# uc-vision/splat-trainer

Measured on AMD Instinct MI355X. Metric: fwd+bwd Gaussians/s, higher is better.
Workload: dtype f32

## Files before the change

### splat-trainer_amd/csrc/composite.hip

```cpp
#include "gsr_device.h"
#include "gsr_dpp_reduce.h"
#include "../../include/gsplat_hip.h"

namespace {

inline GsrRasterParams to_params(const GsrRasterParamsC* c) {
  GsrRasterParams rp;
  __builtin_memcpy(&rp, c, sizeof(rp));
  return rp;
}

typedef float v2f __attribute__((ext_vector_type(2)));
struct __attribute__((packed, aligned(4))) Rank4 { uint32_t x, y, z, w; };
#define GSR_V2(x) ((v2f){(x), (x)})

__device__ __forceinline__ v2f eval_q2(v2f dx, float dy, float A, float B, float C) {
#pragma clang fp contract(off)
  const float t = (B + B) * dy;
  const float u = (C * dy) * dy;
  return __builtin_elementwise_fma(dx * A, dx, __builtin_elementwise_fma(GSR_V2(t), dx, GSR_V2(u)));
}
__device__ __forceinline__ void eval_qt(v2f dx, float dy, float A, float B, float C, v2f& q, v2f& tx, v2f& ty) {
#pragma clang fp contract(off)
  const float bdy = B * dy, cdy = C * dy;
  tx = __builtin_elementwise_fma(dx, GSR_V2(A), GSR_V2(bdy));
  ty = __builtin_elementwise_fma(dx, GSR_V2(B), GSR_V2(cdy));
  q = eval_q2(dx, dy, A, B, C);
}
__device__ __forceinline__ v2f eval_alpha2(v2f q, float l2op) {
#pragma clang fp contract(off)
  const v2f e = __builtin_elementwise_fma(q, GSR_V2(-0.72134752044448170368f), GSR_V2(l2op));
  return (v2f){__builtin_amdgcn_exp2f(e.x), __builtin_amdgcn_exp2f(e.y)};
}
__device__ __forceinline__ v2f eval_G2(v2f q) {
#pragma clang fp contract(off)
  const v2f e = q * -0.72134752044448170368f;
  return (v2f){__builtin_amdgcn_exp2f(e.x), __builtin_amdgcn_exp2f(e.y)};
}

__device__ __forceinline__ v2f clamp_alpha2(v2f a, float cmax) {
  return (v2f){__builtin_amdgcn_fmed3f(a.x, 0.f, cmax), __builtin_amdgcn_fmed3f(a.y, 0.f, cmax)};
}

struct Splat {
  float u, v, A, B, C, op, qlim, f0, f1, f2, depth, l2op;
  uint32_t halves;
};

template <int C, bool DEPTH = false>
__device__ __forceinline__ Splat load_splat_packed(const float* __restrict__ rec, uint32_t packed) {
  const uint32_t k = packed & 0x3FFFFFFFu;
  const float4* r = reinterpret_cast<const float4*>(rec + (size_t)GSR_ROW_FLOATS * k);
  const float4 r0 = r[0], r1 = r[1];
  Splat s;
  s.u = r0.x; s.v = r0.y; s.A = r0.z; s.B = r0.w; s.C = r1.x; s.op = r1.y; s.qlim = r1.z; s.f0 = r1.w;
  s.f1 = 0.f; s.f2 = 0.f; s.depth = 0.f; s.l2op = 0.f;
  s.halves = packed >> 30;
  if (C > 1 || DEPTH) { const float4 r2 = r[2]; s.f1 = r2.x; s.f2 = r2.y; s.depth = r2.z; s.l2op = r2.w; }
  return s;
}

template <int C, bool DEPTH = false>
__device__ __forceinline__ Splat load_splat(const float* __restrict__ rec, const uint32_t* __restrict__ sorted_rank,
                                            uint32_t i) {
  const uint32_t packed = (uint32_t)__builtin_amdgcn_readfirstlane((int)sorted_rank[i]);
  const uint32_t k = packed & 0x3FFFFFFFu;
  const float4* r = reinterpret_cast<const float4*>(rec + (size_t)GSR_ROW_FLOATS * k);
  const float4 r0 = r[0], r1 = r[1];
  Splat s;
  s.u = r0.x; s.v = r0.y; s.A = r0.z; s.B = r0.w; s.C = r1.x; s.op = r1.y; s.qlim = r1.z; s.f0 = r1.w;
  s.f1 = 0.f; s.f2 = 0.f; s.depth = 0.f; s.l2op = 0.f;
  s.halves = packed >> 30;
  if (C > 1 || DEPTH) { const float4 r2 = r[2]; s.f1 = r2.x; s.f2 = r2.y; s.depth = r2.z; s.l2op = r2.w; }
  return s;
}

#define GSR_SEG_HEAVY 0x80000000u

struct SegDev {
  const uint32_t* tile_seg;
  const uint32_t* seg_desc;
  const uint32_t* seg_total;
  const uint32_t* tile_order;
  float* seg_P;
  float4* seg_TC;
  int* seg_last;
  float* seg_median;
};

#define GSR_TILE_CLASSES 32
#define GSR_TILE_GROUP 16
#define GSR_SEG_CLASS_COUNT(band) (16u + GSR_TILE_CLASSES * (band))
__host__ __device__ inline int gsr_tile_band(int t, int n) { (void)n; return (t / GSR_TILE_GROUP) & 7; }
__host__ __device__ inline int gsr_tile_band_stride(int n) {
  return (n + 8 * GSR_TILE_GROUP - 1) / (8 * GSR_TILE_GROUP) * GSR_TILE_GROUP;
}

__device__ __forceinline__ int ordered_tile(const SegDev& seg, int num_tiles, uint32_t b, int lane) {
  const uint32_t band = b & 7u, t = b >> 3;
  uint32_t upto = lane < GSR_TILE_CLASSES ? seg.seg_total[GSR_SEG_CLASS_COUNT(band) + (GSR_TILE_CLASSES - 1 - lane)] : 0u;
#pragma unroll
  for (int o = 1; o < GSR_TILE_CLASSES; o <<= 1) {
    const uint32_t below = (uint32_t)__shfl_up((int)upto, o, 64);
    if (lane >= o) upto += below;
  }
  const uint64_t longer = __ballot(lane < GSR_TILE_CLASSES && t < upto);
  if (longer == 0ull) return -1;
  const int l = __builtin_ctzll(longer);
  const uint32_t before = l ? (uint32_t)__builtin_amdgcn_readlane((int)upto, l - 1) : 0u;
  return (int)seg.tile_order[((size_t)band * GSR_TILE_CLASSES + (size_t)(GSR_TILE_CLASSES - 1 - l)) *
                                 (size_t)gsr_tile_band_stride(num_tiles) + (t - before)];
}

template <int C>
struct FwdPix {
  v2f T2[2], col2[2][3], med2[2];
  int lastc[4];
  uint32_t pf_rank, pf_bits, pf_sink;
};

constexpr int GSR_K6_PREFETCH = 32;
template <int C, bool PF>
__device__ __forceinline__ void fwd_prefetch_init(FwdPix<C>& px, const uint32_t* __restrict__ sorted_rank,
                                                  uint32_t tile_start, uint32_t begin, uint32_t pf_end, int lane) {
  px.pf_bits = 0u; px.pf_sink = 0u; px.pf_rank = 0u;
  if (!PF) return;
  const uint32_t first = tile_start + ((begin - tile_start + GSR_K6_PREFETCH - 1u) & ~(uint32_t)(GSR_K6_PREFETCH - 1));
  const uint32_t p = first + GSR_K6_PREFETCH + (uint32_t)lane;
  if (lane < GSR_K6_PREFETCH && p < pf_end) px.pf_rank = sorted_rank[p];
}
template <int C>
__device__ __forceinline__ void fwd_prefetch_step(FwdPix<C>& px, const float* __restrict__ rec,
                                                  const uint32_t* __restrict__ sorted_rank, uint32_t i, uint32_t pf_end,
                                                  int lane) {
  px.pf_sink |= px.pf_bits;
  const uint32_t p1 = i + GSR_K6_PREFETCH + (uint32_t)lane, p2 = p1 + GSR_K6_PREFETCH;
  const bool mine = lane < GSR_K6_PREFETCH;
  px.pf_bits = (mine && p1 < pf_end)
                   ? __float_as_uint(rec[(size_t)GSR_ROW_FLOATS * (px.pf_rank & 0x3FFFFFFFu)]) : 0u;
  px.pf_rank = (mine && p2 < pf_end) ? sorted_rank[p2] : 0u;
}

template <int C, bool VIS, bool MEDIAN, bool PF>
__device__ __forceinline__ void fwd_walk(FwdPix<C>& px, const float* __restrict__ rec,
                                         const uint32_t* __restrict__ sorted_rank,
                                         const uint32_t* __restrict__ sorted_inst, uint32_t tile_start, uint32_t begin,
                                         uint32_t end, float fx0, float fy0, const GsrRasterParams& rp, int lane,
                                         float* __restrict__ vis_partial, float* __restrict__ pair_vis,
                                         uint32_t pf_end) {
  const uint32_t vis_slot = (uint32_t)(((lane >> 4) & 1) * 2 + (lane >> 5));
  if (begin >= end) return;
  uint32_t rk[4] = {0u, 0u, 0u, 0u}, rk_next[4] = {0u, 0u, 0u, 0u};
  Splat nxt;
  if constexpr (PF) {
    const Rank4 q4 = *reinterpret_cast<const Rank4*>(sorted_rank + begin);
    rk[0] = (uint32_t)__builtin_amdgcn_readfirstlane((int)q4.x); rk[1] = (uint32_t)__builtin_amdgcn_readfirstlane((int)q4.y);
    rk[2] = (uint32_t)__builtin_amdgcn_readfirstlane((int)q4.z); rk[3] = (uint32_t)__builtin_amdgcn_readfirstlane((int)q4.w);
    nxt = load_splat_packed<C, MEDIAN>(rec, rk[0]);
  } else {
    nxt = load_splat<C, MEDIAN>(rec, sorted_rank, begin);
  }
  for (uint32_t i = begin; i < end; i += 4) {
    if (PF && ((i - tile_start) & (GSR_K6_PREFETCH - 1)) == 0u) fwd_prefetch_step<C>(px, rec, sorted_rank, i, pf_end, lane);
    if constexpr (PF) {
      if (i + 4 < end) {
        const Rank4 q4 = *reinterpret_cast<const Rank4*>(sorted_rank + i + 4);
        rk_next[0] = (uint32_t)__builtin_amdgcn_readfirstlane((int)q4.x); rk_next[1] = (uint32_t)__builtin_amdgcn_readfirstlane((int)q4.y);
        rk_next[2] = (uint32_t)__builtin_amdgcn_readfirstlane((int)q4.z); rk_next[3] = (uint32_t)__builtin_amdgcn_readfirstlane((int)q4.w);
      }
    }
    float wq[4] = {0.f, 0.f, 0.f, 0.f};
#pragma unroll
    for (int m = 0; m < 4; ++m) {
      if (i + m < end) {
        const Splat s = nxt;
        if constexpr (PF) {
          if (i + m + 1 < end) nxt = load_splat_packed<C, MEDIAN>(rec, m < 3 ? rk[m + 1] : rk_next[0]);
        } else {
          nxt = load_splat<C, MEDIAN>(rec, sorted_rank, min(i + m + 1, end - 1u));
        }
        const v2f dx2 = (v2f){fx0, fx0 + 8.f} - GSR_V2(s.u);
        const int idx = (int)(i - tile_start) + m + 1;
        v2f wsum2 = GSR_V2(0.f);
#pragma unroll
        for (int h = 0; h < 2; ++h) {
          if (!(s.halves & (1u << h))) continue;
          const float dy = (h ? fy0 + 8.f : fy0) - s.v;
          const v2f q = eval_q2(dx2, dy, s.A, s.B, s.C);
          const bool hit0 = px.T2[h].x >= rp.T_eps && q.x <= s.qlim;
          const bool hit1 = px.T2[h].y >= rp.T_eps && q.y <= s.qlim;
          if (__ballot(hit0 || hit1) != 0ull) {
            const v2f G = eval_G2(q);
            const v2f a_raw = G * s.op;
            v2f alpha = clamp_alpha2(a_raw, rp.clamp_max_alpha);
            alpha = (v2f){hit0 ? alpha.x : 0.f, hit1 ? alpha.y : 0.f};
            const v2f w = alpha * px.T2[h];
            px.col2[h][0] = __builtin_elementwise_fma(w, GSR_V2(s.f0), px.col2[h][0]);
            if (C > 1) px.col2[h][1] = __builtin_elementwise_fma(w, GSR_V2(s.f1), px.col2[h][1]);
            if (C > 2) px.col2[h][2] = __builtin_elementwise_fma(w, GSR_V2(s.f2), px.col2[h][2]);
            wsum2 += w;
            px.T2[h] = px.T2[h] - w;
            if (hit0) px.lastc[2 * h] = idx;
            if (hit1) px.lastc[2 * h + 1] = idx;
            if (MEDIAN) {
              if (hit0 && px.med2[h].x == 0.f && px.T2[h].x < 0.5f) px.med2[h].x = s.depth;
              if (hit1 && px.med2[h].y == 0.f && px.T2[h].y < 0.5f) px.med2[h].y = s.depth;
            }
          }
        }
        wq[m] = wsum2.x + wsum2.y;
      }
    }
    if (VIS) {
      float r = gsr_swap16_add(gsr_swap32_add(wq[0], wq[1]), gsr_swap32_add(wq[2], wq[3]));
      r = gsr_row_sum_to_lane15(r);
      const uint32_t pos = i + vis_slot;
      if ((lane & 15) == 15 && pos < end) {
        pair_vis[pos] = r;
        if (r > 0.f) vis_partial[sorted_inst[pos]] = r;
      }
    }
    const bool live = px.T2[0].x >= rp.T_eps || px.T2[0].y >= rp.T_eps || px.T2[1].x >= rp.T_eps ||
                      px.T2[1].y >= rp.T_eps;
    if (__ballot(live) == 0ull) break;
    if constexpr (PF) { rk[0] = rk_next[0]; rk[1] = rk_next[1]; rk[2] = rk_next[2]; rk[3] = rk_next[3]; }
  }
}

template <int C>
__device__ __forceinline__ void fwd_init(FwdPix<C>& px, int px0, int py0, int W, int H) {
#pragma unroll
  for (int h = 0; h < 2; ++h) {
    const bool in_y = (py0 + 8 * h) < H;
    px.T2[h] = (v2f){(in_y && px0 < W) ? 1.f : 0.f, (in_y && (px0 + 8) < W) ? 1.f : 0.f};
    px.med2[h] = GSR_V2(0.f);
    px.col2[h][0] = px.col2[h][1] = px.col2[h][2] = GSR_V2(0.f);
  }
#pragma unroll
  for (int p = 0; p < 4; ++p) px.lastc[p] = 0;
}

template <int C>
__device__ __forceinline__ void seg_alpha_pass(uint32_t sidx, const float* __restrict__ rec,
                                               const uint32_t* __restrict__ sorted_rank, int tiles_x,
                                               const GsrRasterParams& rp, const SegDev& seg) {
  const uint32_t* d = seg.seg_desc + 4 * (size_t)sidx;
  const int tile = (int)d[0];
  const uint32_t begin = d[1], end = d[2];
  const int lane = (int)threadIdx.x;
  const int tx = tile % tiles_x, ty = tile / tiles_x;
  const float fx0 = (float)(tx * 16 + (lane & 7)) + 0.5f, fy0 = (float)(ty * 16 + (lane >> 3)) + 0.5f;
  v2f P2[2] = {GSR_V2(1.f), GSR_V2(1.f)};
  Splat nxt = load_splat<1>(rec, sorted_rank, begin);
  for (uint32_t i = begin; i < end; ++i) {
    const Splat s = nxt;
    if (i + 1 < end) nxt = load_splat<1>(rec, sorted_rank, i + 1);
    const v2f dx2 = (v2f){fx0, fx0 + 8.f} - GSR_V2(s.u);
#pragma unroll
    for (int h = 0; h < 2; ++h) {
      if (!(s.halves & (1u << h))) continue;
      const float dy = (h ? fy0 + 8.f : fy0) - s.v;
      const v2f q = eval_q2(dx2, dy, s.A, s.B, s.C);
      const bool in0 = q.x <= s.qlim, in1 = q.y <= s.qlim;
      if (__ballot(in0 || in1) != 0ull) {
        v2f alpha = clamp_alpha2(eval_G2(q) * s.op, rp.clamp_max_alpha);
        alpha = (v2f){in0 ? alpha.x : 0.f, in1 ? alpha.y : 0.f};
        P2[h] = P2[h] - alpha * P2[h];
      }
    }
  }
  float* out = seg.seg_P + 256 * (size_t)sidx + lane;
  out[0] = P2[0].x; out[64] = P2[0].y; out[128] = P2[1].x; out[192] = P2[1].y;
}

template <int C, bool VIS, bool MEDIAN, bool PF>
__global__ __launch_bounds__(64) void composite_fwd_kernel(const float* __restrict__ rec,
                                                           const uint32_t* __restrict__ sorted_rank,
                                                           const uint32_t* __restrict__ sorted_inst,
                                                           const uint32_t* __restrict__ tile_range, int W, int H,
                                                           int tiles_x, int num_tiles, GsrRasterParams rp,
                                                           float* __restrict__ image, float* __restrict__ final_T,
                                                           int* __restrict__ last, float* __restrict__ median,
                                                           float* __restrict__ vis_partial,
                                                           float* __restrict__ pair_vis, SegDev seg, int tile_blocks) {
  if ((int)blockIdx.x >= tile_blocks) {
    const uint32_t h = blockIdx.x - (uint32_t)tile_blocks;
    if (h < seg.seg_total[1]) {
      const uint32_t sidx = (seg.tile_seg + 2 * (size_t)num_tiles)[h];
      if (sidx != 0xFFFFFFFFu) {
        const uint32_t* d = seg.seg_desc + 4 * (size_t)sidx;
        if (d[1] < d[2]) seg_alpha_pass<C>(sidx, rec, sorted_rank, tiles_x, rp, seg);
      }
    }
    return;
  }
  const int lane = (int)threadIdx.x;
  int tile;
  if (seg.tile_order) {
    tile = ordered_tile(seg, num_tiles, blockIdx.x, lane);
    if (tile < 0) return;
  } else {
    tile = gsr_xcd_remap((int)blockIdx.x, num_tiles);
  }
  const uint32_t tseg = seg.tile_seg ? seg.tile_seg[2 * tile + 1] : 0u;
  if (tseg & GSR_SEG_HEAVY) return;
  const int tx = tile % tiles_x, ty = tile / tiles_x;
  const int px0 = tx * 16 + (lane & 7), py0 = ty * 16 + (lane >> 3);
  const float fx0 = (float)px0 + 0.5f, fy0 = (float)py0 + 0.5f;
  const uint32_t start = tile_range[2 * tile], end = tile_range[2 * tile + 1];

  FwdPix<C> px;
  fwd_init<C>(px, px0, py0, W, H);
  fwd_prefetch_init<C, PF>(px, sorted_rank, start, start, end, lane);
  if (tseg == 0u) {
    fwd_walk<C, VIS, MEDIAN, PF>(px, rec, sorted_rank, sorted_inst, start, start, end, fx0, fy0, rp, lane, vis_partial,
                             pair_vis, end);
  } else {
    const uint32_t first = seg.tile_seg[2 * tile];
    for (uint32_t j = 0; j < tseg; ++j) {
      const uint32_t* d = seg.seg_desc + 4 * (size_t)(first + j);
      fwd_walk<C, VIS, MEDIAN, PF>(px, rec, sorted_rank, sorted_inst, start, d[1], d[2], fx0, fy0, rp, lane, vis_partial,
                               pair_vis, end);
      float4* out = seg.seg_TC + 256 * (size_t)(first + j) + lane;
#pragma unroll
      for (int p = 0; p < 4; ++p) {
        const int h = p >> 1;
        out[64 * p] = (p & 1) ? make_float4(px.T2[h].y, px.col2[h][0].y, px.col2[h][1].y, px.col2[h][2].y)
                              : make_float4(px.T2[h].x, px.col2[h][0].x, px.col2[h][1].x, px.col2[h][2].x);
      }
      const bool live = px.T2[0].x >= rp.T_eps || px.T2[0].y >= rp.T_eps || px.T2[1].x >= rp.T_eps ||
                        px.T2[1].y >= rp.T_eps;
      if (__ballot(live) == 0ull) break;
    }
  }

  if (PF && (px.pf_sink | px.pf_bits) == 0x7FC0FFEEu) final_T[0] = 0.f;
#pragma unroll
  for (int p = 0; p < 4; ++p) {
    const int x = px0 + 8 * (p & 1), y = py0 + 8 * (p >> 1);
    if (x < W && y < H) {
      const size_t pix = (size_t)y * W + x;
      const int h = p >> 1;
#pragma unroll
      for (int c = 0; c < C; ++c) image[pix * C + c] = (p & 1) ? px.col2[h][c].y : px.col2[h][c].x;
      final_T[pix] = (p & 1) ? px.T2[h].y : px.T2[h].x;
      last[pix] = px.lastc[p];
      if (MEDIAN) median[pix] = (p & 1) ? px.med2[h].y : px.med2[h].x;
    }
  }
}

template <int C, bool VIS, bool MEDIAN, bool PF>
__global__ __launch_bounds__(64) void seg_composite_kernel(const float* __restrict__ rec,
                                                           const uint32_t* __restrict__ sorted_rank,
                                                           const uint32_t* __restrict__ sorted_inst,
                                                           const uint32_t* __restrict__ tile_range, int W, int H,
                                                           int tiles_x, int num_tiles, GsrRasterParams rp,
                                                           float* __restrict__ vis_partial,
                                                           float* __restrict__ pair_vis, SegDev seg) {
  if (blockIdx.x >= seg.seg_total[1]) return;
  const uint32_t sidx = (seg.tile_seg + 2 * (size_t)num_tiles)[blockIdx.x];
  if (sidx == 0xFFFFFFFFu) return;
  const uint32_t* d = seg.seg_desc + 4 * (size_t)sidx;
  const int tile = (int)d[0];
  const uint32_t begin = d[1], end = d[2];
  const uint32_t first = seg.tile_seg[2 * tile];
  const int lane = (int)threadIdx.x;
  const int tx = tile % tiles_x, ty = tile / tiles_x;
  const int px0 = tx * 16 + (lane & 7), py0 = ty * 16 + (lane >> 3);
  const float fx0 = (float)px0 + 0.5f, fy0 = (float)py0 + 0.5f;

  FwdPix<C> px;
  fwd_init<C>(px, px0, py0, W, H);
  fwd_prefetch_init<C, PF>(px, sorted_rank, tile_range[2 * tile], begin, end, lane);
  for (uint32_t s = first; s < sidx; ++s) {
    const float* P = seg.seg_P + 256 * (size_t)s + lane;
    px.T2[0] = px.T2[0] * (v2f){P[0], P[64]};
    px.T2[1] = px.T2[1] * (v2f){P[128], P[192]};
  }
  const bool alive[4] = {px.T2[0].x >= rp.T_eps, px.T2[0].y >= rp.T_eps, px.T2[1].x >= rp.T_eps, px.T2[1].y >= rp.T_eps};
  if (__ballot(alive[0] || alive[1] || alive[2] || alive[3]) != 0ull)
    fwd_walk<C, VIS, MEDIAN, PF>(px, rec, sorted_rank, sorted_inst, tile_range[2 * tile], begin, end, fx0, fy0, rp, lane,
                             vis_partial, pair_vis, end);
  const size_t o = 256 * (size_t)sidx + lane;
#pragma unroll
  for (int p = 0; p < 4; ++p) {
    const int h = p >> 1;
    const float t = (p & 1) ? px.T2[h].y : px.T2[h].x;
    seg.seg_TC[o + 64 * p] = (p & 1) ? make_float4(alive[p] ? t : -1.f, px.col2[h][0].y, px.col2[h][1].y, px.col2[h][2].y)
                                     : make_float4(alive[p] ? t : -1.f, px.col2[h][0].x, px.col2[h][1].x, px.col2[h][2].x);
    seg.seg_last[o + 64 * p] = px.lastc[p];
    if (MEDIAN) seg.seg_median[o + 64 * p] = (p & 1) ? px.med2[h].y : px.med2[h].x;
  }
}

template <int C, bool MEDIAN>
__global__ __launch_bounds__(64) void seg_combine_kernel(int W, int H, int tiles_x, int num_tiles,
                                                         float* __restrict__ image, float* __restrict__ final_T,
                                                         int* __restrict__ last, float* __restrict__ median,
                                                         SegDev seg) {
  const int tile = (int)blockIdx.x;
  const uint32_t tseg = seg.tile_seg[2 * tile + 1];
  if (!(tseg & GSR_SEG_HEAVY)) return;
  const uint32_t n = tseg & ~GSR_SEG_HEAVY;
  const uint32_t first = seg.tile_seg[2 * tile];
  const int lane = (int)threadIdx.x;
  const int tx = tile % tiles_x, ty = tile / tiles_x;
  const int px0 = tx * 16 + (lane & 7), py0 = ty * 16 + (lane >> 3);
  float col[4][3], T[4], med[4];
  int lastc[4];
#pragma unroll
  for (int p = 0; p < 4; ++p) {
    col[p][0] = col[p][1] = col[p][2] = 0.f;
    T[p] = 1.f; med[p] = 0.f; lastc[p] = 0;
  }
  for (uint32_t j = 0; j < n; ++j) {
    const size_t s = first + j, o = 256 * s + lane;
#pragma unroll
    for (int p = 0; p < 4; ++p) {
      const float4 tc = seg.seg_TC[o + 64 * p];
      if (tc.x >= 0.f) T[p] = tc.x;
      const int l = seg.seg_last[o + 64 * p];
      if (l != 0) lastc[p] = l;
      if (MEDIAN) {
        const float m = seg.seg_median[o + 64 * p];
        if (med[p] == 0.f && m != 0.f) med[p] = m;
      }
      col[p][0] += tc.y; col[p][1] += tc.z; col[p][2] += tc.w;
      seg.seg_TC[o + 64 * p] = make_float4(tc.x, col[p][0], col[p][1], col[p][2]);
    }
  }
#pragma unroll
  for (int p = 0; p < 4; ++p) {
    const int x = px0 + 8 * (p & 1), y = py0 + 8 * (p >> 1);
    if (x < W && y < H) {
      const size_t pix = (size_t)y * W + x;
#pragma unroll
      for (int c = 0; c < C; ++c) image[pix * C + c] = col[p][c];
      final_T[pix] = T[p];
      last[pix] = lastc[p];
      if (MEDIAN) median[pix] = med[p];
    }
  }
}

constexpr int GSR_K7_WAVES = 6;
constexpr int GSR_K7_SEG_GROUP_LOG2 = 5;
template <int C>
__global__ __launch_bounds__(64) __attribute__((amdgpu_waves_per_eu(GSR_K7_WAVES, GSR_K7_WAVES))) void composite_bwd_kernel(const float* __restrict__ rec,
                                                           const uint32_t* __restrict__ sorted_rank,
                                                           const uint32_t* __restrict__ sorted_inst,
                                                           const float* __restrict__ pair_vis,
                                                           const uint32_t* __restrict__ tile_range, int W, int H,
                                                           int tiles_x, int num_tiles, GsrRasterParams rp,
                                                           const float* __restrict__ final_T,
                                                           const int* __restrict__ last,
                                                           const float* __restrict__ dL_dimage,
                                                           const float* __restrict__ image,
                                                           float* __restrict__ partial, SegDev seg,
                                                           uint32_t seg_capacity, uint32_t seg_blocks) {
  int tile, lo = 0, seg_hi = 0x7fffffff;
  uint32_t sidx = 0u;
  const bool is_seg = blockIdx.x < seg_blocks;
  if (is_seg) {
    sidx = gsr_xcd_group_remap(blockIdx.x, GSR_K7_SEG_GROUP_LOG2);
    if (sidx >= min(seg.seg_total[0], seg_capacity)) return;
    const uint32_t* d = seg.seg_desc + 4 * (size_t)sidx;
    tile = (int)d[0];
    const uint32_t tstart = tile_range[2 * tile];
    lo = (int)(d[1] - tstart);
    seg_hi = (int)(d[2] - tstart);
  } else {
    const uint32_t b = blockIdx.x - seg_blocks;
    if (seg.tile_order) {
      tile = ordered_tile(seg, num_tiles, b, (int)threadIdx.x);
      if (tile < 0) return;
    } else {
      if ((int)b >= num_tiles) return;
      tile = gsr_xcd_remap((int)b, num_tiles);
    }
    if (seg.tile_seg && seg.tile_seg[2 * tile + 1] != 0u) return;
  }
  const int lane = (int)threadIdx.x;
  const int tx = tile % tiles_x, ty = tile / tiles_x;
  const int px0 = tx * 16 + (lane & 7), py0 = ty * 16 + (lane >> 3);
  const float fx0 = (float)px0 + 0.5f, fy0 = (float)py0 + 0.5f;
  const uint32_t start = tile_range[2 * tile];

  v2f T2[2], g2[2][3], ga2[2];
  int lastc[4];
  int tile_last = 0;
#pragma unroll
  for (int h = 0; h < 2; ++h) {
    T2[h] = GSR_V2(1.f); ga2[h] = GSR_V2(0.f);
    g2[h][0] = g2[h][1] = g2[h][2] = GSR_V2(0.f);
  }
#pragma unroll
  for (int p = 0; p < 4; ++p) {
    const int px = px0 + 8 * (p & 1), py = py0 + 8 * (p >> 1);
    const int h = p >> 1;
    lastc[p] = 0;
    if (px < W && py < H) {
      const size_t pix = (size_t)py * W + px;
      float t = final_T[pix];
      float4 tc = make_float4(0.f, 0.f, 0.f, 0.f);
      if (is_seg) {
        tc = seg.seg_TC[256 * (size_t)sidx + 64 * p + lane];
        t = tc.x < 0.f ? 1.f : tc.x;
      }
      const float upto[3] = {tc.y, tc.z, tc.w};
      if (p & 1) T2[h].y = t; else T2[h].x = t;
      lastc[p] = last[pix];
      float gb = 0.f;
#pragma unroll
      for (int c = 0; c < C; ++c) {
        const float gv = dL_dimage[pix * C + c];
        if (p & 1) g2[h][c].y = gv; else g2[h][c].x = gv;
        if (is_seg) gb = fmaf(gv, image[pix * C + c] - upto[c], gb);
      }
      if (p & 1) ga2[h].y = gb; else ga2[h].x = gb;
    }
    tile_last = max(tile_last, lastc[p]);
  }
#pragma unroll
  for (int o = 32; o > 0; o >>= 1) tile_last = max(tile_last, __shfl_xor(tile_last, o, 64));
  tile_last = __builtin_amdgcn_readfirstlane(tile_last);
  const int hi = min(tile_last, seg_hi);
  if (hi <= lo) return;
  __shared__ float red[12 * 80];
  const int rslot = lane < 44 ? (lane >> 2) * 68 + (lane & 3) * 16 : 0;

  for (int cbase = lo + (((hi - lo - 1) >> 6) << 6); cbase >= lo; cbase -= 64) {
    const int n = min(64, hi - cbase);
    const uint32_t li = start + (uint32_t)cbase + (uint32_t)lane;
    const float pv = (lane < n) ? pair_vis[li] : 0.f;
    const int my_rank = (lane < n) ? (int)sorted_rank[li] : 0;
    const int my_inst = (lane < n) ? (int)sorted_inst[li] : 0;
    uint64_t flags = __ballot(pv > 0.f);
    if (flags == 0ull) continue;
    int j = 63 - __builtin_clzll(flags);
    Splat nxt = load_splat_packed<C, true>(rec, (uint32_t)__builtin_amdgcn_readlane(my_rank, j));
    uint32_t inst_nxt = (uint32_t)__builtin_amdgcn_readlane(my_inst, j);
    while (true) {
      const Splat s = nxt;
      const uint32_t inst_j = inst_nxt;
      const int pos = cbase + j;
      flags &= ~(1ull << j);
      const bool more = flags != 0ull;
      if (more) {
        j = 63 - __builtin_clzll(flags);
        nxt = load_splat_packed<C, true>(rec, (uint32_t)__builtin_amdgcn_readlane(my_rank, j));
        inst_nxt = (uint32_t)__builtin_amdgcn_readlane(my_inst, j);
      }
      const v2f dx2 = (v2f){fx0, fx0 + 8.f} - GSR_V2(s.u);
      v2f mx2 = GSR_V2(0.f), my2 = mx2, mxx2 = mx2, mxy2 = mx2, myy2 = mx2, dop2 = mx2, prune2 = mx2, split2 = mx2;
      v2f df2[3] = {mx2, mx2, mx2};
#pragma unroll
      for (int h = 0; h < 2; ++h) {
        if (!(s.halves & (1u << h))) continue;
        const float dy = (h ? fy0 + 8.f : fy0) - s.v;
        v2f q, tx_, ty_;
        eval_qt(dx2, dy, s.A, s.B, s.C, q, tx_, ty_);
        const bool hit0 = pos < lastc[2 * h] && q.x <= s.qlim;
        const bool hit1 = pos < lastc[2 * h + 1] && q.y <= s.qlim;
        if (__ballot(hit0 || hit1) != 0ull) {
          const v2f a_raw = eval_alpha2(q, s.l2op);
          v2f alpha = clamp_alpha2(a_raw, rp.clamp_max_alpha);
          alpha = (v2f){hit0 ? alpha.x : 0.f, hit1 ? alpha.y : 0.f};
          const v2f om = GSR_V2(1.f) - alpha;
          const v2f inv = {__builtin_amdgcn_rcpf(om.x), __builtin_amdgcn_rcpf(om.y)};
          const v2f Tb = T2[h] * inv;
          T2[h] = Tb;
          const v2f w = alpha * Tb;
          v2f gc = g2[h][0] * s.f0;
          if (C > 1) gc = __builtin_elementwise_fma(g2[h][1], GSR_V2(s.f1), gc);
          if (C > 2) gc = __builtin_elementwise_fma(g2[h][2], GSR_V2(s.f2), gc);
          df2[0] = __builtin_elementwise_fma(w, g2[h][0], df2[0]);
          if (C > 1) df2[1] = __builtin_elementwise_fma(w, g2[h][1], df2[1]);
          if (C > 2) df2[2] = __builtin_elementwise_fma(w, g2[h][2], df2[2]);
          const v2f dLda = Tb * gc - ga2[h] * inv;
          ga2[h] = __builtin_elementwise_fma(gc, w, ga2[h]);
          prune2 = (v2f){__builtin_fmaf(__builtin_fabsf(dLda.x), alpha.x, prune2.x),
                         __builtin_fmaf(__builtin_fabsf(dLda.y), alpha.y, prune2.y)};
          const bool m0 = hit0 && a_raw.x <= rp.clamp_max_alpha;
          const bool m1 = hit1 && a_raw.y <= rp.clamp_max_alpha;
          v2f GdG = a_raw * dLda;
          GdG = (v2f){m0 ? GdG.x : 0.f, m1 ? GdG.y : 0.f};
          dop2 += GdG;
          const v2f px_ = GdG * dx2, py_ = GdG * dy;
          mx2 += px_;
          my2 += py_;
          mxx2 = __builtin_elementwise_fma(px_, dx2, mxx2);
          mxy2 = __builtin_elementwise_fma(px_, GSR_V2(dy), mxy2);
          myy2 = __builtin_elementwise_fma(py_, GSR_V2(dy), myy2);
          const v2f nn = __builtin_elementwise_fma(ty_, ty_, tx_ * tx_);
          split2 = (v2f){__builtin_fmaf(__builtin_fabsf(GdG.x), __builtin_amdgcn_sqrtf(nn.x), split2.x),
                         __builtin_fmaf(__builtin_fabsf(GdG.y), __builtin_amdgcn_sqrtf(nn.y), split2.y)};
        }
      }
      float du = mx2.x + mx2.y, dv = my2.x + my2.y, dA = mxx2.x + mxx2.y, dB = mxy2.x + mxy2.y, dC = myy2.x + myy2.y;
      float dop = dop2.x + dop2.y, prune = prune2.x + prune2.y, split = split2.x + split2.y;
      float df[3] = {df2[0].x + df2[0].y, df2[1].x + df2[1].y, df2[2].x + df2[2].y};
      {
        asm volatile("s_mov_b32 m0, %11\n"
                     "s_nop 0\n"
                     "ds_write_addtid_b32 %0 offset:0\n"
                     "ds_write_addtid_b32 %1 offset:272\n"
                     "ds_write_addtid_b32 %2 offset:544\n"
                     "ds_write_addtid_b32 %3 offset:816\n"
                     "ds_write_addtid_b32 %4 offset:1088\n"
                     "ds_write_addtid_b32 %5 offset:1360\n"
                     "ds_write_addtid_b32 %6 offset:1632\n"
                     "ds_write_addtid_b32 %7 offset:1904\n"
                     "ds_write_addtid_b32 %8 offset:2176\n"
                     "ds_write_addtid_b32 %9 offset:2448\n"
                     "ds_write_addtid_b32 %10 offset:2720\n"
                     :: "v"(du), "v"(dv), "v"(dA), "v"(dB), "v"(dC), "v"(dop), "v"(prune), "v"(split), "v"(df[0]), "v"(df[1]),
                        "v"(df[2]), "s"((uint32_t)(uintptr_t)red) : "memory");
        gsr_wave_lds_fence();
        const float4* rd = reinterpret_cast<const float4*>(red + rslot);
        const float4 a = rd[0], b = rd[1], c = rd[2], d = rd[3];
        gsr_wave_lds_fence();
        const v2f t = (((v2f){a.x, a.y} + (v2f){a.z, a.w}) + ((v2f){b.x, b.y} + (v2f){b.z, b.w})) +
                      (((v2f){c.x, c.y} + (v2f){c.z, c.w}) + ((v2f){d.x, d.y} + (v2f){d.z, d.w}));
        float tot = t.x + t.y;
        asm volatile("s_nop 1\n"
                     "v_add_f32_dpp %0, %0, %0 quad_perm:[1,0,3,2] row_mask:0xf bank_mask:0xf\n"
                     "s_nop 1\n"
                     "v_add_f32_dpp %0, %0, %0 quad_perm:[2,3,0,1] row_mask:0xf bank_mask:0xf\n"
                     : "+v"(tot));
        if (lane < 44 && (lane & 3) == 0) partial[(size_t)GSR_PARTIAL_FLOATS * inst_j + (lane >> 2)] = tot;
      }
      if (!more) break;
    }
  }
}

__host__ __device__ inline void segment_thresholds(int32_t seg_cfg, int32_t heavy_cfg, int64_t O, int32_t num_tiles,
                                                   int32_t needs_grad, int32_t wide, uint32_t* seg_out,
                                                   uint32_t* heavy_out) {
  if (O < 0) O = 0;
  int64_t heavy = heavy_cfg > 0 ? (int64_t)heavy_cfg : 120 + O / 2900;
  if (heavy_cfg <= 0 && heavy < 512) heavy = 512;
  int64_t seg;
  if (seg_cfg > 0) {
    seg = seg_cfg;
  } else {
    if (needs_grad && wide) {
      seg = 256;
    } else if (needs_grad) {
      const int64_t per = 6 * (int64_t)(num_tiles > 0 ? num_tiles : 1);
      seg = (O / per + 3) & ~(int64_t)3;
      seg = seg < 64 ? 64 : (seg > 256 ? 256 : seg);
    } else {
      seg = (heavy / 2) & ~(int64_t)3;
      if (seg < 256) seg = 256;
    }
    seg = (seg + 3) & ~(int64_t)3;
    if (seg < 4) seg = 4;
  }
  *seg_out = (uint32_t)seg;
  *heavy_out = (uint32_t)(heavy > seg ? heavy : seg);
}

__global__ __launch_bounds__(256) void segment_plan_kernel(const uint32_t* __restrict__ tile_range, int num_tiles,
                                                           int32_t seg_cfg, int32_t heavy_cfg, int32_t needs_grad,
                                                           int32_t wide, int64_t O,
                                                           const uint32_t* __restrict__ O_dev,
                                                           uint32_t capacity, uint32_t heavy_capacity,
                                                           uint32_t* __restrict__ tile_seg,
                                                           uint32_t* __restrict__ seg_desc,
                                                           uint32_t* __restrict__ seg_total,
                                                           uint32_t* __restrict__ tile_order) {
  const int t = (int)(blockIdx.x * blockDim.x + threadIdx.x);
  __shared__ uint32_t s_count[8 * GSR_TILE_CLASSES], s_base[8 * GSR_TILE_CLASSES];
  static_assert(8 * GSR_TILE_CLASSES == 256, "one LDS counter per thread of the block");
  s_count[threadIdx.x] = 0u;
  __syncthreads();
  bool filed = false;
  uint32_t key = 0u, local = 0u;
  if (t < num_tiles) {
    uint32_t seg_pairs, heavy_min;
    const int64_t O_now = O_dev ? (int64_t)*O_dev : O;
    segment_thresholds(seg_cfg, heavy_cfg, O_now, num_tiles, needs_grad, wide, &seg_pairs, &heavy_min);
    const uint32_t a = tile_range[2 * t], len = tile_range[2 * t + 1] - a;
    bool heavy = len > heavy_min;
    const uint32_t seg_heavy = max(seg_pairs, min(256u, (heavy_min / 2u) & ~3u));
    const uint32_t seg_t = heavy ? max(seg_heavy, (((len + 127u) / 128u) + 3u) & ~3u) : seg_pairs;
    uint32_t n = len > seg_pairs ? (len + seg_t - 1) / seg_t : 0u;
    uint32_t at = 0u;
    if (n) {
      at = atomicAdd(seg_total, n);
      if (at + n > capacity) {
        for (uint32_t j = at; j < capacity; ++j) {
          uint32_t* d = seg_desc + 4 * (size_t)j;
          d[0] = (uint32_t)t; d[1] = a; d[2] = a; d[3] = 0u;
        }
        n = 0u;
      }
    }
    if (n && heavy) {
      const uint32_t hat = atomicAdd(seg_total + 1, n);
      if (hat + n <= heavy_capacity) {
        uint32_t* list = tile_seg + 2 * (size_t)num_tiles;
        for (uint32_t j = 0; j < n; ++j) list[hat + j] = at + j;
      } else {
        heavy = false;
        uint32_t* list = tile_seg + 2 * (size_t)num_tiles;
        for (uint32_t j = hat; j < heavy_capacity; ++j) list[j] = 0xFFFFFFFFu;
      }
    }
    tile_seg[2 * t] = at;
    tile_seg[2 * t + 1] = n | ((n && heavy) ? GSR_SEG_HEAVY : 0u);
    if (tile_order && !(n && heavy)) {
      const uint32_t mean = (uint32_t)max((int64_t)1, O_now / num_tiles);
      const uint32_t cls = min((uint32_t)(GSR_TILE_CLASSES - 1), len * 8u / mean);
      key = (uint32_t)gsr_tile_band(t, num_tiles) * GSR_TILE_CLASSES + cls;
      local = atomicAdd(&s_count[key], 1u);
      filed = true;
    }
    for (uint32_t j = 0; j < n; ++j) {
      uint32_t* d = seg_desc + 4 * (size_t)(at + j);
      d[0] = (uint32_t)t; d[1] = a + j * seg_t; d[2] = min(a + (j + 1) * seg_t, a + len); d[3] = j;
    }
  }
  __syncthreads();
  if (s_count[threadIdx.x])
    s_base[threadIdx.x] = atomicAdd(seg_total + GSR_SEG_CLASS_COUNT(0) + threadIdx.x, s_count[threadIdx.x]);
  __syncthreads();
  if (filed)
    tile_order[(size_t)key * (size_t)gsr_tile_band_stride(num_tiles) + s_base[key] + local] = (uint32_t)t;
}

inline SegDev to_segdev(const GsrSegmentsC* sg) {
  SegDev d;
  if (sg) {
    d.tile_seg = sg->tile_seg; d.seg_desc = sg->seg_desc; d.seg_total = sg->seg_total; d.seg_P = sg->seg_P;
    d.tile_order = sg->tile_order;
    d.seg_TC = reinterpret_cast<float4*>(sg->seg_TC); d.seg_last = sg->seg_last; d.seg_median = sg->seg_median;
  } else {
    d.tile_seg = nullptr; d.seg_desc = nullptr; d.seg_total = nullptr; d.seg_P = nullptr; d.seg_TC = nullptr;
    d.tile_order = nullptr;
    d.seg_last = nullptr; d.seg_median = nullptr;
  }
  return d;
}

inline bool seg_ok(const GsrSegmentsC* sg, bool median) {
  if (!sg) return true;
  if (sg->capacity <= 0 || sg->heavy_capacity < 0 || sg->heavy_capacity > sg->capacity) return false;
  return sg->tile_seg && sg->seg_desc && sg->seg_total && sg->seg_P && sg->seg_TC && sg->seg_last &&
         (!median || sg->seg_median);
}

}

#include "composite_wide.inc"

extern "C" {

int gsr_segment_thresholds_wide(int32_t seg_pairs_cfg, int32_t heavy_min_cfg, int64_t O, int32_t num_tiles,
                                int32_t needs_grad, int32_t wide, int32_t* seg_pairs_out, int32_t* heavy_min_out) {
  if (!seg_pairs_out || !heavy_min_out || num_tiles <= 0) return GSR_ERR_INVALID_ARGUMENT;
  uint32_t seg, heavy;
  segment_thresholds(seg_pairs_cfg, heavy_min_cfg, O, num_tiles, needs_grad, wide, &seg, &heavy);
  *seg_pairs_out = (int32_t)seg;
  *heavy_min_out = (int32_t)heavy;
  return GSR_OK;
}

int gsr_segment_thresholds(int32_t seg_pairs_cfg, int32_t heavy_min_cfg, int64_t O, int32_t num_tiles, int32_t needs_grad,
// ... 150 lines not shown
```

Measured before the change: 550.7 million.

## Batch visibility writes via LDS, use scalar constant loads, hoist backward pixel loads

The forward walk now buffers per-quad visibility sums in a small LDS park and writes pair_vis and vis_partial once per 64-entry block as coalesced stores, instead of scattered per-quad stores. Table lookups (tile_order, seg_desc, seg_total, tile_seg) go through constant address space so they can become scalar loads, and segment descriptors are prefetched one iteration ahead. In the backward kernel, pixel inputs are loaded unconditionally with clamped coordinates and grouped before use, and the per-chunk rank/inst loads drop their lane predication. The reduction LDS array is shrunk and m0 is declared clobbered. These changes add LDS fences and extra loads for out-of-bounds pixels in exchange.

```diff
diff --git a/splat-trainer_amd/csrc/composite.hip b/splat-trainer_amd/csrc/composite.hip
--- a/splat-trainer_amd/csrc/composite.hip
+++ b/splat-trainer_amd/csrc/composite.hip
@@ -13,6 +13,15 @@
 typedef float v2f __attribute__((ext_vector_type(2)));
 struct __attribute__((packed, aligned(4))) Rank4 { uint32_t x, y, z, w; };
 #define GSR_V2(x) ((v2f){(x), (x)})
+typedef float v3f __attribute__((ext_vector_type(3)));
+typedef float v4f __attribute__((ext_vector_type(4)));
+template <int C> struct ChanVec;
+template <> struct ChanVec<1> { typedef float type; };
+template <> struct ChanVec<2> { typedef v2f type; };
+template <> struct ChanVec<3> { typedef v3f type; };
+__device__ __forceinline__ float chan(float v, int) { return v; }
+__device__ __forceinline__ float chan(v2f v, int c) { return v[c]; }
+__device__ __forceinline__ float chan(v3f v, int c) { return v[c]; }
 
 __device__ __forceinline__ v2f eval_q2(v2f dx, float dy, float A, float B, float C) {
 #pragma clang fp contract(off)
@@ -77,6 +86,10 @@
 
 #define GSR_SEG_HEAVY 0x80000000u
 
+__device__ __forceinline__ uint32_t load_table_word(const uint32_t* p) {
+  return *(const __attribute__((address_space(4))) uint32_t*)p;
+}
+
 struct SegDev {
   const uint32_t* tile_seg;
   const uint32_t* seg_desc;
@@ -108,8 +121,8 @@
   if (longer == 0ull) return -1;
   const int l = __builtin_ctzll(longer);
   const uint32_t before = l ? (uint32_t)__builtin_amdgcn_readlane((int)upto, l - 1) : 0u;
-  return (int)seg.tile_order[((size_t)band * GSR_TILE_CLASSES + (size_t)(GSR_TILE_CLASSES - 1 - l)) *
-                                 (size_t)gsr_tile_band_stride(num_tiles) + (t - before)];
+  return (int)load_table_word(seg.tile_order + ((size_t)band * GSR_TILE_CLASSES + (size_t)(GSR_TILE_CLASSES - 1 - l)) *
+                                                   (size_t)gsr_tile_band_stride(num_tiles) + (t - before));
 }
 
 template <int C>
@@ -147,9 +160,10 @@
                                          const uint32_t* __restrict__ sorted_inst, uint32_t tile_start, uint32_t begin,
                                          uint32_t end, float fx0, float fy0, const GsrRasterParams& rp, int lane,
                                          float* __restrict__ vis_partial, float* __restrict__ pair_vis,
-                                         uint32_t pf_end) {
+                                         uint32_t pf_end, float* vis_park) {
   const uint32_t vis_slot = (uint32_t)(((lane >> 4) & 1) * 2 + (lane >> 5));
   if (begin >= end) return;
+  float* const park = vis_park + vis_slot;
   uint32_t rk[4] = {0u, 0u, 0u, 0u}, rk_next[4] = {0u, 0u, 0u, 0u};
   Splat nxt;
   if constexpr (PF) {
@@ -160,70 +174,84 @@
   } else {
     nxt = load_splat<C, MEDIAN>(rec, sorted_rank, begin);
   }
-  for (uint32_t i = begin; i < end; i += 4) {
-    if (PF && ((i - tile_start) & (GSR_K6_PREFETCH - 1)) == 0u) fwd_prefetch_step<C>(px, rec, sorted_rank, i, pf_end, lane);
-    if constexpr (PF) {
-      if (i + 4 < end) {
-        const Rank4 q4 = *reinterpret_cast<const Rank4*>(sorted_rank + i + 4);
-        rk_next[0] = (uint32_t)__builtin_amdgcn_readfirstlane((int)q4.x); rk_next[1] = (uint32_t)__builtin_amdgcn_readfirstlane((int)q4.y);
-        rk_next[2] = (uint32_t)__builtin_amdgcn_readfirstlane((int)q4.z); rk_next[3] = (uint32_t)__builtin_amdgcn_readfirstlane((int)q4.w);
-      }
-    }
-    float wq[4] = {0.f, 0.f, 0.f, 0.f};
-#pragma unroll
-    for (int m = 0; m < 4; ++m) {
-      if (i + m < end) {
-        const Splat s = nxt;
-        if constexpr (PF) {
-          if (i + m + 1 < end) nxt = load_splat_packed<C, MEDIAN>(rec, m < 3 ? rk[m + 1] : rk_next[0]);
-        } else {
-          nxt = load_splat<C, MEDIAN>(rec, sorted_rank, min(i + m + 1, end - 1u));
+  for (uint32_t blk = begin; blk < end; blk += 64) {
+    const uint32_t blk_end = min(blk + 64u, end);
+    uint32_t blk_inst = 0u;
+    if (VIS) blk_inst = sorted_inst[min(blk + (uint32_t)lane, blk_end - 1u)];
+    bool dead = false;
+    uint32_t i = blk;
+    for (; i < blk_end; i += 4) {
+      if (PF && ((i - tile_start) & (GSR_K6_PREFETCH - 1)) == 0u) fwd_prefetch_step<C>(px, rec, sorted_rank, i, pf_end, lane);
+      if constexpr (PF) {
+        if (i + 4 < end) {
+          const Rank4 q4 = *reinterpret_cast<const Rank4*>(sorted_rank + i + 4);
+          rk_next[0] = (uint32_t)__builtin_amdgcn_readfirstlane((int)q4.x); rk_next[1] = (uint32_t)__builtin_amdgcn_readfirstlane((int)q4.y);
+          rk_next[2] = (uint32_t)__builtin_amdgcn_readfirstlane((int)q4.z); rk_next[3] = (uint32_t)__builtin_amdgcn_readfirstlane((int)q4.w);
         }
-        const v2f dx2 = (v2f){fx0, fx0 + 8.f} - GSR_V2(s.u);
-        const int idx = (int)(i - tile_start) + m + 1;
-        v2f wsum2 = GSR_V2(0.f);
-#pragma unroll
-        for (int h = 0; h < 2; ++h) {
-          if (!(s.halves & (1u << h))) continue;
-          const float dy = (h ? fy0 + 8.f : fy0) - s.v;
-          const v2f q = eval_q2(dx2, dy, s.A, s.B, s.C);
-          const bool hit0 = px.T2[h].x >= rp.T_eps && q.x <= s.qlim;
-          const bool hit1 = px.T2[h].y >= rp.T_eps && q.y <= s.qlim;
-          if (__ballot(hit0 || hit1) != 0ull) {
-            const v2f G = eval_G2(q);
-            const v2f a_raw = G * s.op;
-            v2f alpha = clamp_alpha2(a_raw, rp.clamp_max_alpha);
-            alpha = (v2f){hit0 ? alpha.x : 0.f, hit1 ? alpha.y : 0.f};
-            const v2f w = alpha * px.T2[h];
-            px.col2[h][0] = __builtin_elementwise_fma(w, GSR_V2(s.f0), px.col2[h][0]);
-            if (C > 1) px.col2[h][1] = __builtin_elementwise_fma(w, GSR_V2(s.f1), px.col2[h][1]);
-            if (C > 2) px.col2[h][2] = __builtin_elementwise_fma(w, GSR_V2(s.f2), px.col2[h][2]);
-            wsum2 += w;
-            px.T2[h] = px.T2[h] - w;
-            if (hit0) px.lastc[2 * h] = idx;
-            if (hit1) px.lastc[2 * h + 1] = idx;
-            if (MEDIAN) {
-              if (hit0 && px.med2[h].x == 0.f && px.T2[h].x < 0.5f) px.med2[h].x = s.depth;
-              if (hit1 && px.med2[h].y == 0.f && px.T2[h].y < 0.5f) px.med2[h].y = s.depth;
+      }
+      float wq[4] = {0.f, 0.f, 0.f, 0.f};
+#pragma unroll
+      for (int m = 0; m < 4; ++m) {
+        if (i + m < end) {
+          const Splat s = nxt;
+          if constexpr (PF) {
+            if (i + m + 1 < end) nxt = load_splat_packed<C, MEDIAN>(rec, m < 3 ? rk[m + 1] : rk_next[0]);
+          } else {
+            nxt = load_splat<C, MEDIAN>(rec, sorted_rank, min(i + m + 1, end - 1u));
+          }
+          const v2f dx2 = (v2f){fx0, fx0 + 8.f} - GSR_V2(s.u);
+          const int idx = (int)(i - tile_start) + m + 1;
+          v2f wsum2 = GSR_V2(0.f);
+#pragma unroll
+          for (int h = 0; h < 2; ++h) {
+            if (!(s.halves & (1u << h))) continue;
+            const float dy = (h ? fy0 + 8.f : fy0) - s.v;
+            const v2f q = eval_q2(dx2, dy, s.A, s.B, s.C);
+            const bool hit0 = px.T2[h].x >= rp.T_eps && q.x <= s.qlim;
+            const bool hit1 = px.T2[h].y >= rp.T_eps && q.y <= s.qlim;
+            if (__ballot(hit0 || hit1) != 0ull) {
+              const v2f G = eval_G2(q);
+              const v2f a_raw = G * s.op;
+              v2f alpha = clamp_alpha2(a_raw, rp.clamp_max_alpha);
+              alpha = (v2f){hit0 ? alpha.x : 0.f, hit1 ? alpha.y : 0.f};
+              const v2f w = alpha * px.T2[h];
+              px.col2[h][0] = __builtin_elementwise_fma(w, GSR_V2(s.f0), px.col2[h][0]);
+              if (C > 1) px.col2[h][1] = __builtin_elementwise_fma(w, GSR_V2(s.f1), px.col2[h][1]);
+              if (C > 2) px.col2[h][2] = __builtin_elementwise_fma(w, GSR_V2(s.f2), px.col2[h][2]);
+              wsum2 += w;
+              px.T2[h] = px.T2[h] - w;
+              if (hit0) px.lastc[2 * h] = idx;
+              if (hit1) px.lastc[2 * h + 1] = idx;
+              if (MEDIAN) {
+                if (hit0 && px.med2[h].x == 0.f && px.T2[h].x < 0.5f) px.med2[h].x = s.depth;
+                if (hit1 && px.med2[h].y == 0.f && px.T2[h].y < 0.5f) px.med2[h].y = s.depth;
+              }
             }
           }
+          wq[m] = wsum2.x + wsum2.y;
         }
-        wq[m] = wsum2.x + wsum2.y;
-      }
+      }
+      if (VIS) {
+        float r = gsr_swap16_add(gsr_swap32_add(wq[0], wq[1]), gsr_swap32_add(wq[2], wq[3]));
+        r = gsr_row_sum_to_lane15(r);
+        if ((lane & 15) == 15) park[i - blk] = r;
+      }
+      const bool live = px.T2[0].x >= rp.T_eps || px.T2[0].y >= rp.T_eps || px.T2[1].x >= rp.T_eps ||
+                        px.T2[1].y >= rp.T_eps;
+      if (__ballot(live) == 0ull) { dead = true; i += 4; break; }
+      if constexpr (PF) { rk[0] = rk_next[0]; rk[1] = rk_next[1]; rk[2] = rk_next[2]; rk[3] = rk_next[3]; }
     }
     if (VIS) {
-      float r = gsr_swap16_add(gsr_swap32_add(wq[0], wq[1]), gsr_swap32_add(wq[2], wq[3]));
-      r = gsr_row_sum_to_lane15(r);
-      const uint32_t pos = i + vis_slot;
-      if ((lane & 15) == 15 && pos < end) {
-        pair_vis[pos] = r;
-        if (r > 0.f) vis_partial[sorted_inst[pos]] = r;
-      }
-    }
-    const bool live = px.T2[0].x >= rp.T_eps || px.T2[0].y >= rp.T_eps || px.T2[1].x >= rp.T_eps ||
-                      px.T2[1].y >= rp.T_eps;
-    if (__ballot(live) == 0ull) break;
-    if constexpr (PF) { rk[0] = rk_next[0]; rk[1] = rk_next[1]; rk[2] = rk_next[2]; rk[3] = rk_next[3]; }
+      gsr_wave_lds_fence();
+      const float r = vis_park[lane];
+      gsr_wave_lds_fence();
+      asm volatile("" : "+v"(blk_inst));
+      if (blk + (uint32_t)lane < min(i, blk_end)) {
+        if (r > 0.f) vis_partial[blk_inst] = r;
+        pair_vis[blk + (uint32_t)lane] = r;
+      }
+    }
+    if (dead) break;
   }
 }
 
@@ -309,18 +337,23 @@
   const float fx0 = (float)px0 + 0.5f, fy0 = (float)py0 + 0.5f;
   const uint32_t start = tile_range[2 * tile], end = tile_range[2 * tile + 1];
 
+  __shared__ float vis_park[64];
   FwdPix<C> px;
   fwd_init<C>(px, px0, py0, W, H);
   fwd_prefetch_init<C, PF>(px, sorted_rank, start, start, end, lane);
   if (tseg == 0u) {
     fwd_walk<C, VIS, MEDIAN, PF>(px, rec, sorted_rank, sorted_inst, start, start, end, fx0, fy0, rp, lane, vis_partial,
-                             pair_vis, end);
+                             pair_vis, end, vis_park);
   } else {
-    const uint32_t first = seg.tile_seg[2 * tile];
-    for (uint32_t j = 0; j < tseg; ++j) {
-      const uint32_t* d = seg.seg_desc + 4 * (size_t)(first + j);
-      fwd_walk<C, VIS, MEDIAN, PF>(px, rec, sorted_rank, sorted_inst, start, d[1], d[2], fx0, fy0, rp, lane, vis_partial,
-                               pair_vis, end);
+    const uint32_t first = (uint32_t)__builtin_amdgcn_readfirstlane((int)seg.tile_seg[2 * tile]);
+    const uint32_t* d = seg.seg_desc + 4 * (size_t)first;
+    uint32_t seg_begin = load_table_word(d + 1), seg_end = load_table_word(d + 2);
+    for (uint32_t j = 0; j < tseg; ++j, d += 4) {
+      uint32_t next_begin = seg_begin, next_end = seg_end;
+      if (j + 1 < tseg) { next_begin = load_table_word(d + 5); next_end = load_table_word(d + 6); }
+      fwd_walk<C, VIS, MEDIAN, PF>(px, rec, sorted_rank, sorted_inst, start, seg_begin, seg_end, fx0, fy0, rp, lane,
+                                   vis_partial, pair_vis, end, vis_park);
+      seg_begin = next_begin; seg_end = next_end;
       float4* out = seg.seg_TC + 256 * (size_t)(first + j) + lane;
 #pragma unroll
       for (int p = 0; p < 4; ++p) {
@@ -370,6 +403,7 @@
   const int px0 = tx * 16 + (lane & 7), py0 = ty * 16 + (lane >> 3);
   const float fx0 = (float)px0 + 0.5f, fy0 = (float)py0 + 0.5f;
 
+  __shared__ float vis_park[64];
   FwdPix<C> px;
   fwd_init<C>(px, px0, py0, W, H);
   fwd_prefetch_init<C, PF>(px, sorted_rank, tile_range[2 * tile], begin, end, lane);
@@ -381,7 +415,7 @@
   const bool alive[4] = {px.T2[0].x >= rp.T_eps, px.T2[0].y >= rp.T_eps, px.T2[1].x >= rp.T_eps, px.T2[1].y >= rp.T_eps};
   if (__ballot(alive[0] || alive[1] || alive[2] || alive[3]) != 0ull)
     fwd_walk<C, VIS, MEDIAN, PF>(px, rec, sorted_rank, sorted_inst, tile_range[2 * tile], begin, end, fx0, fy0, rp, lane,
-                             vis_partial, pair_vis, end);
+                             vis_partial, pair_vis, end, vis_park);
   const size_t o = 256 * (size_t)sidx + lane;
 #pragma unroll
   for (int p = 0; p < 4; ++p) {
@@ -464,12 +498,12 @@
   const bool is_seg = blockIdx.x < seg_blocks;
   if (is_seg) {
     sidx = gsr_xcd_group_remap(blockIdx.x, GSR_K7_SEG_GROUP_LOG2);
-    if (sidx >= min(seg.seg_total[0], seg_capacity)) return;
+    if (sidx >= min(load_table_word(seg.seg_total), seg_capacity)) return;
     const uint32_t* d = seg.seg_desc + 4 * (size_t)sidx;
-    tile = (int)d[0];
+    tile = (int)load_table_word(d);
     const uint32_t tstart = tile_range[2 * tile];
-    lo = (int)(d[1] - tstart);
-    seg_hi = (int)(d[2] - tstart);
+    lo = (int)(load_table_word(d + 1) - tstart);
+    seg_hi = (int)(load_table_word(d + 2) - tstart);
   } else {
     const uint32_t b = blockIdx.x - seg_blocks;
     if (seg.tile_order) {
@@ -479,7 +513,7 @@
       if ((int)b >= num_tiles) return;
       tile = gsr_xcd_remap((int)b, num_tiles);
     }
-    if (seg.tile_seg && seg.tile_seg[2 * tile + 1] != 0u) return;
+    if (seg.tile_seg && load_table_word(seg.tile_seg + 2 * tile + 1) != 0u) return;
   }
   const int lane = (int)threadIdx.x;
   const int tx = tile % tiles_x, ty = tile / tiles_x;
@@ -495,31 +529,53 @@
     T2[h] = GSR_V2(1.f); ga2[h] = GSR_V2(0.f);
     g2[h][0] = g2[h][1] = g2[h][2] = GSR_V2(0.f);
   }
+  v4f tc[4];
+  typename ChanVec<C>::type img[4], g_in[4];
+  float t_in[4];
+  int last_in[4];
+  size_t pixc[4];
 #pragma unroll
   for (int p = 0; p < 4; ++p) {
-    const int px = px0 + 8 * (p & 1), py = py0 + 8 * (p >> 1);
+    const int px = min(px0 + 8 * (p & 1), W - 1), py = min(py0 + 8 * (p >> 1), H - 1);
+    pixc[p] = (size_t)py * W + px;
+    tc[p] = (v4f){0.f, 0.f, 0.f, 0.f};
+    img[p] = 0.f;
+  }
+  if (is_seg) {
+#pragma unroll
+    for (int p = 0; p < 4; ++p) {
+      tc[p] = reinterpret_cast<const v4f*>(seg.seg_TC)[256 * (size_t)sidx + 64 * p + lane];
+      __builtin_memcpy(&img[p], image + pixc[p] * C, sizeof(float) * C);
+    }
+  }
+#pragma unroll
+  for (int p = 0; p < 4; ++p) {
+    t_in[p] = final_T[pixc[p]];
+    last_in[p] = last[pixc[p]];
+    __builtin_memcpy(&g_in[p], dL_dimage + pixc[p] * C, sizeof(float) * C);
+  }
+  asm volatile("" : "+v"(tc[0]), "+v"(tc[1]), "+v"(tc[2]), "+v"(tc[3]), "+v"(img[0]), "+v"(img[1]), "+v"(img[2]),
+                    "+v"(img[3]), "+v"(g_in[0]), "+v"(g_in[1]), "+v"(g_in[2]), "+v"(g_in[3]), "+v"(t_in[0]),
+                    "+v"(t_in[1]), "+v"(t_in[2]), "+v"(t_in[3]), "+v"(last_in[0]), "+v"(last_in[1]), "+v"(last_in[2]),
+                    "+v"(last_in[3]));
+#pragma unroll
+  for (int p = 0; p < 4; ++p) {
+    const bool inside = (px0 + 8 * (p & 1)) < W && (py0 + 8 * (p >> 1)) < H;
     const int h = p >> 1;
-    lastc[p] = 0;
-    if (px < W && py < H) {
-      const size_t pix = (size_t)py * W + px;
-      float t = final_T[pix];
-      float4 tc = make_float4(0.f, 0.f, 0.f, 0.f);
-      if (is_seg) {
-        tc = seg.seg_TC[256 * (size_t)sidx + 64 * p + lane];
-        t = tc.x < 0.f ? 1.f : tc.x;
-      }
-      const float upto[3] = {tc.y, tc.z, tc.w};
-      if (p & 1) T2[h].y = t; else T2[h].x = t;
-      lastc[p] = last[pix];
-      float gb = 0.f;
-#pragma unroll
-      for (int c = 0; c < C; ++c) {
-        const float gv = dL_dimage[pix * C + c];
-        if (p & 1) g2[h][c].y = gv; else g2[h][c].x = gv;
-        if (is_seg) gb = fmaf(gv, image[pix * C + c] - upto[c], gb);
-      }
-      if (p & 1) ga2[h].y = gb; else ga2[h].x = gb;
-    }
+    float t = t_in[p];
+    if (is_seg) t = tc[p].x < 0.f ? 1.f : tc[p].x;
+    const float upto[3] = {tc[p].y, tc[p].z, tc[p].w};
+    t = inside ? t : 1.f;
+    if (p & 1) T2[h].y = t; else T2[h].x = t;
+    lastc[p] = inside ? last_in[p] : 0;
+    float gb = 0.f;
+#pragma unroll
+    for (int c = 0; c < C; ++c) {
+      const float gv = inside ? chan(g_in[p], c) : 0.f;
+      if (p & 1) g2[h][c].y = gv; else g2[h][c].x = gv;
+      if (is_seg) gb = fmaf(gv, chan(img[p], c) - upto[c], gb);
+    }
+    if (p & 1) ga2[h].y = gb; else ga2[h].x = gb;
     tile_last = max(tile_last, lastc[p]);
   }
 #pragma unroll
@@ -527,16 +583,17 @@
   tile_last = __builtin_amdgcn_readfirstlane(tile_last);
   const int hi = min(tile_last, seg_hi);
   if (hi <= lo) return;
-  __shared__ float red[12 * 80];
+  __shared__ float red[11 * 68];
   const int rslot = lane < 44 ? (lane >> 2) * 68 + (lane & 3) * 16 : 0;
 
   for (int cbase = lo + (((hi - lo - 1) >> 6) << 6); cbase >= lo; cbase -= 64) {
     const int n = min(64, hi - cbase);
-    const uint32_t li = start + (uint32_t)cbase + (uint32_t)lane;
-    const float pv = (lane < n) ? pair_vis[li] : 0.f;
-    const int my_rank = (lane < n) ? (int)sorted_rank[li] : 0;
-    const int my_inst = (lane < n) ? (int)sorted_inst[li] : 0;
-    uint64_t flags = __ballot(pv > 0.f);
+    const uint32_t li = start + (uint32_t)cbase + (uint32_t)min(lane, n - 1);
+    float pv = pair_vis[li];
+    int my_rank = (int)sorted_rank[li];
+    int my_inst = (int)sorted_inst[li];
+    asm volatile("" : "+v"(pv), "+v"(my_rank), "+v"(my_inst));
+    uint64_t flags = __ballot(lane < n && pv > 0.f);
     if (flags == 0ull) continue;
     int j = 63 - __builtin_clzll(flags);
     Splat nxt = load_splat_packed<C, true>(rec, (uint32_t)__builtin_amdgcn_readlane(my_rank, j));
@@ -602,6 +659,8 @@
       float dop = dop2.x + dop2.y, prune = prune2.x + prune2.y, split = split2.x + split2.y;
       float df[3] = {df2[0].x + df2[0].y, df2[1].x + df2[1].y, df2[2].x + df2[2].y};
       {
+#pragma clang diagnostic push
+#pragma clang diagnostic ignored "-Winline-asm"
         asm volatile("s_mov_b32 m0, %11\n"
                      "s_nop 0\n"
                      "ds_write_addtid_b32 %0 offset:0\n"
@@ -616,7 +675,8 @@
                      "ds_write_addtid_b32 %9 offset:2448\n"
                      "ds_write_addtid_b32 %10 offset:2720\n"
                      :: "v"(du), "v"(dv), "v"(dA), "v"(dB), "v"(dC), "v"(dop), "v"(prune), "v"(split), "v"(df[0]), "v"(df[1]),
-                        "v"(df[2]), "s"((uint32_t)(uintptr_t)red) : "memory");
+                        "v"(df[2]), "s"((uint32_t)(uintptr_t)red) : "memory", "m0");
+#pragma clang diagnostic pop
         gsr_wave_lds_fence();
         const float4* rd = reinterpret_cast<const float4*>(red + rslot);
         const float4 a = rd[0], b = rd[1], c = rd[2], d = rd[3];
```

After: 562.9 million, median of 6. +2.2%, better.
